# ay-lab/fithic

Measured on AMD Instinct MI355X. Metric: contact-pairs/sec through spline+p-value+BH pass (5 kb cis, whole node), higher is better.
Workload: dtype f64

## Files before the change

### fithic_amd/_capi.py

```python
import ctypes
import os
import subprocess

import numpy as np

from . import _loader

_PKG = os.path.dirname(os.path.abspath(__file__))
LIB_PATH = _loader.LIB_PATH
CSRC = os.path.join(_PKG, "csrc")

FHX_OK = 0
FHX_ERR_ARG, FHX_ERR_NO_DEVICE, FHX_ERR_HIP, FHX_ERR_UNSUPPORTED, FHX_ERR_REFERENCE_EXIT, FHX_ERR_NOMEM, FHX_ERR_INTERNAL = -1, -2, -3, -4, -5, -6, -7
MODE_INTRA_ONLY, MODE_INTER_ONLY, MODE_ALL = 0, 1, 2
TOTALS_REFERENCE, TOTALS_WIDE = 0, 1
INT64_MAX = (1 << 63) - 1

(A_HIST_SUMCC, A_HIST_NPAIRS, A_BIN_LB, A_BIN_UB, A_BIN_POSS, A_BIN_SUMCC, A_BIN_SUMDIST, A_BIN_POSS7, A_X, A_Y,
 A_KNOTS, A_COEFFS, A_TABLE_X, A_TABLE_Y0, A_TABLE_Y, A_OUTLIER_DIST_HIST, A_FDR_COUNTS, A_BIN_POSS0, A_DIST_KEYS,
 A_OUTLIER_DISTS) = range(20)
_ARRAY_DTYPE = {A_BIN_SUMDIST: np.float64, A_X: np.float64, A_Y: np.float64, A_KNOTS: np.float64,
                A_COEFFS: np.float64, A_TABLE_Y0: np.float64, A_TABLE_Y: np.float64}


# ... 71 lines not shown
    "fhx_set_skip_limit": (ctypes.c_int, [_P, ctypes.c_int64]),
    "fhx_next_pass": (ctypes.c_int, [_P, _I64P]),
    "fhx_reset_passes": (ctypes.c_int, [_P]),
    "fhx_get_stats": (ctypes.c_int, [_P, ctypes.POINTER(FhxStats)]),
    "fhx_fetch": (ctypes.c_int, [_P, _F64P, _F64P, _F64P, _F64P, _F64P]),
    "fhx_fetch_flags": (ctypes.c_int, [_P, ctypes.POINTER(ctypes.c_uint8), ctypes.POINTER(ctypes.c_uint8)]),
    "fhx_fetch_outlier_rows": (ctypes.c_int, [_P, ctypes.POINTER(ctypes.c_int64), ctypes.c_int64, ctypes.POINTER(ctypes.c_int64)]),
    "fhx_get_array": (ctypes.c_int, [_P, ctypes.c_int, _P, ctypes.c_int64, _I64P]),
    "fhx_device_ptr": (_P, [_P, ctypes.c_int]),
    "fhx_n_sorted": (ctypes.c_int64, [_P]),
    "fhx_bh_sort_stats": (ctypes.c_int, [_P, _I64P]),
    "fhx_k3_pass_info": (ctypes.c_int, [_P, _I64P]),
    "fhx_debug_k3_tiles_per_group": (ctypes.c_int, [_P, ctypes.c_int]),
    "fhx_debug_device_blocks": (ctypes.c_int, [_I64P, _I64P]),
    "fhx_debug_k1_wide": (ctypes.c_int, [_P, ctypes.c_int]),
    "fhx_k3_compact_variant": (ctypes.c_int, [_P, ctypes.POINTER(ctypes.c_int32)]),
    "fhx_kernel_seconds": (ctypes.c_int, [_P, _F64P, _F64P, _F64P]),
    "fhx_kernel_seconds_total": (ctypes.c_int, [_P, _F64P, _I64P, ctypes.c_int]),
    "fhx_kernel_events_dropped": (ctypes.c_int, [_P, _I64P]),
    "fhx_k2_heavy_launch": (ctypes.c_int, [_P, _F64P, _I64P]),
    "fhx_k2_heavy_clock": (ctypes.c_int, [_P, _F64P]),
    "fhx_k2_class_rows": (ctypes.c_int, [_P, _I64P]),
    "fhx_bdtrc_array": (ctypes.c_int, [_P, ctypes.c_double, _I32P, _F64P, ctypes.c_int64, _F64P]),
    "fhx_debug_format": (ctypes.c_int, [_P, _F64P, ctypes.c_int64, ctypes.c_int32, ctypes.c_char_p, _I32P]),
    "fhx_debug_contfrac": (ctypes.c_int, [_P, ctypes.c_int, ctypes.c_int, _F64P, _F64P, _F64P, ctypes.c_int64, _F64P]),
    "fhx_debug_lean_div": (ctypes.c_int, [_P, _F64P, _F64P, ctypes.c_int64, _F64P]),
    "fhx_debug_table_div": (ctypes.c_int, [_P, ctypes.c_int, _F64P, ctypes.c_int64, _F64P, _I32P]),
    "fhx_debug_classify": (ctypes.c_int, [_P, ctypes.c_double, _I32P, _F64P, ctypes.c_int64, _I32P, _I32P, _F64P]),
    "fhx_debug_k2_rows": (ctypes.c_int, [_P, ctypes.c_double, ctypes.c_double, _I32P, _F64P, ctypes.POINTER(ctypes.c_uint8), ctypes.c_int64,
                                         ctypes.c_int32, _F64P, _I64P, _I64P, _I64P, ctypes.c_int64]),
# ... 652 lines not shown
                        [int(v) for v in n]))

    def k3_pass_info(self):
        n = (ctypes.c_int64 * 8)()
        self._check(self._L.fhx_k3_pass_info(self._h, n))
        v = ctypes.c_int32(0)
        self._check(self._L.fhx_k3_compact_variant(self._h, ctypes.byref(v)))
        return [int(x) for x in n] + [v.value]

    def debug_k3_tiles_per_group(self, per):
        self._check(self._L.fhx_debug_k3_tiles_per_group(self._h, int(per)))

    def debug_k1_wide(self, on):
        self._check(self._L.fhx_debug_k1_wide(self._h, 1 if on else 0))

    def kernel_events_dropped(self):
        n = (ctypes.c_int64 * 4)()
        self._check(self._L.fhx_kernel_events_dropped(self._h, n))
        return list(n)

    def k2_heavy_launch(self):
        sec, rows = ctypes.c_double(0), ctypes.c_int64(0)
        self._check(self._L.fhx_k2_heavy_launch(self._h, ctypes.byref(sec), ctypes.byref(rows)))
        return sec.value, rows.value

    def k2_heavy_clock(self):
        ghz = ctypes.c_double(0)
        self._check(self._L.fhx_k2_heavy_clock(self._h, ctypes.byref(ghz)))
        return ghz.value

# ... 765 lines not shown
```

### fithic_amd/csrc/fhx_ctx.hpp

```cpp
#pragma once
#include <hip/hip_runtime.h>

#include <atomic>
#include <functional>
#include <chrono>
#include <thread>
#include <memory>
#include <sys/stat.h>
#include <unistd.h>
#include <deque>
#include <mutex>
#include <map>
#include <condition_variable>
#include <algorithm>
#include <climits>
#include <cstddef>
#include <cmath>
#include <cstdio>
#include <cstdlib>
#include <cstring>
#include <string>
#include <vector>

#include "../../include/fithic_mi355x.h"
// ... 32 lines not shown
    int32_t nslots;
    int32_t pad;
};

struct K1Sums {
    long long inter_count, inter_sum, intra_all_count, intra_all_sum, in_range_count, in_range_sum, n_skipped;
    int max_count, pad;
};

struct K2Params {
    const int32_t* loc1;
    const int32_t* loc2;
    const int32_t* count;
    const double* slot_bias;
    bool no_bias;
    const double* prior_lut;
    int lut_len;
    dev::BinomTables intra, inter;
    double inter_chr_prob;
    double outlier_thres;
    int lo_idx, hi_idx;
    int mode;
    int64_t n;
    double* p;
    unsigned long long* top_hist;
    uint8_t* outlier;
    int nonfixed;
    const int32_t* slot_mid;
    const double* table_x;
    const double* table_y;
// ... 197 lines not shown
    bool have_params = false;

    FragTable frags;
    bool have_frags = false;
    int n_chr = 0;

    std::vector<int32_t> bias_chr, bias_mid;
    std::vector<double> bias_val;
    bool have_bias = false;

    int64_t n_rows = 0;
    int32_t *d_loc1 = nullptr, *d_loc2 = nullptr, *d_count = nullptr;
    uint32_t* d_k1key = nullptr;
    bool k1key_valid = false;
    bool k1_force_wide = false;
    bool counts_integral = true;
    std::vector<ChrGrid> grid;
    ChrGrid* d_grid = nullptr;
    int16_t* d_slot_chr = nullptr;
    double* d_slot_bias = nullptr;
    int64_t n_slots = 0;
    int64_t n_dist = 0;
    bool tables_dirty = true;

    int pass_no = 0;
    uint8_t *d_skip = nullptr, *d_outlier = nullptr;
    bool skip_active = false;
    unsigned long long *d_hist_cc = nullptr, *d_hist_np = nullptr, *d_out_hist = nullptr;
    DeviceWords* d_words = nullptr;
    K1Sums* d_sums = nullptr;
// ... 140 lines not shown
    return (int)std::max<int64_t>(1, std::min<int64_t>(b, max_blocks));
}

inline int k2_classify_grid(int64_t n) {
    return grid_for(n, K2_CL_TILE, K2_MAX_SHARDS);
}
inline long long k2_shard_capacity(int64_t n) {
    const long long tiles = std::max<long long>(1, (n + K2_CL_TILE - 1) / K2_CL_TILE), grid = k2_classify_grid(n);
    return ((tiles + grid - 1) / grid) * (long long)K2_CL_TILE;
}


int build_slot_tables(fhx_ctx* ctx);
int run_ids(fhx_ctx* ctx, const unsigned long long* keys, int64_t n, unsigned int* ids, unsigned int* tile_scratch, int64_t* n_runs);
int alloc_row_arrays(fhx_ctx* ctx, int64_t n, int64_t n_dist);
int ingest_device_rows_nonfixed(fhx_ctx* ctx, const int32_t* c1, const int32_t* m1, const int32_t* c2, const int32_t* m2,
                                const int32_t* cnt, int64_t n);
int ingest_device_rows(fhx_ctx* ctx, const int32_t* c1, const int32_t* m1, const int32_t* c2, const int32_t* m2, const int32_t* cnt,
                       int64_t n);
int pass_stats_nonfixed(fhx_ctx* ctx, fhx_stats* out);
int launch_k1(fhx_ctx* ctx);
void fold_kernel_events(fhx_ctx* ctx);
void before_rerecord(fhx_ctx* ctx, int group);
K2Params make_k2_params(fhx_ctx* c);
void launch_k2_extras(fhx_ctx* ctx, const K2Params& P, int64_t n_rows, double* d_expcc, double* d_b1, double* d_b2);
int ensure_sort_scratch(fhx_ctx* ctx);
int sort_blocks_for(int64_t n_hint);
int radix_sort_pairs(fhx_ctx* ctx, unsigned long long* keys[2], unsigned int* vals[2], const unsigned long long* counter, int passes,
                     int* result_buf, int64_t n_hint = -1);
void launch_rs_scan(fhx_ctx* ctx, int nblk);
// ... 17 lines not shown
```

### fithic_amd/csrc/fhx_device.hip

```cpp
#include <thread>

#include "fhx_ctx.hpp"

extern "C" {

const char* fhx_version(void) { return "fithic-mi355x 0.2.0 (gfx950)"; }

int fhx_create(int device, fhx_ctx** out) {
    if (!out) return FHX_ERR_ARG;
    *out = nullptr;
    fhx_ctx* ctx = new (std::nothrow) fhx_ctx();
    if (!ctx) return FHX_ERR_NOMEM;
    ctx->device = device;
    if (device >= 0) {
        int count = 0;
        if (hipGetDeviceCount(&count) != hipSuccess || device >= count) {
            delete ctx;
            return FHX_ERR_NO_DEVICE;
        }
        if (hipSetDevice(device) != hipSuccess || hipStreamCreateWithFlags(&ctx->stream, hipStreamNonBlocking) != hipSuccess) {
            delete ctx;
            return FHX_ERR_HIP;
        }
        for (auto& e : ctx->ev)
// ... 25 lines not shown
void fhx_destroy(fhx_ctx* ctx) {
    if (!ctx) return;
    if (ctx->sig_sorter) fhx_destroy(ctx->sig_sorter);
    ctx->sig_sorter = nullptr;
    (void)fhx_comm_destroy(ctx);
    if (ctx->device >= 0) {
        (void)hipSetDevice(ctx->device);
        if (ctx->stream) (void)hipStreamSynchronize(ctx->stream);
        fhx_ingest_contacts_discard(ctx);
        fhx_pinned_pair_free(ctx->pinned);
        ctx->pinned = nullptr;
        dev_free(ctx->d_loc1);
        dev_free(ctx->d_loc2);
        dev_free(ctx->d_count);
        dev_free(ctx->d_k1key);
        dev_free(ctx->d_grid);
        dev_free(ctx->d_slot_chr);
        dev_free(ctx->d_slot_bias);
        dev_free(ctx->d_skip);
        dev_free(ctx->d_outlier);
        dev_free(ctx->d_grow);
        dev_free(ctx->d_hist_cc);
        dev_free(ctx->d_hist_np);
        dev_free(ctx->d_out_hist);
        dev_free(ctx->d_words);
        dev_free(ctx->d_sums);
        dev_free(ctx->d_fit_tables);
        if (ctx->h_fit_stage) (void)hipHostFree(ctx->h_fit_stage);
        if (ctx->ev_fit_copy) (void)hipEventDestroy(ctx->ev_fit_copy);
        if (ctx->ev_k3) (void)hipEventDestroy(ctx->ev_k3);
// ... 24 lines not shown
    delete ctx;
}

const char* fhx_last_error(fhx_ctx* ctx) { return ctx ? ctx->err.c_str() : "null context"; }

int fhx_set_params(fhx_ctx* ctx, const fhx_params* p) {
    if (!ctx || !p) return FHX_ERR_ARG;
    if (p->resolution < 0) return fail(ctx, FHX_ERR_ARG, "resolution must be >= 0 (0 = non-fixed-size data)");
    if (p->resolution > INT32_MAX) return fail(ctx, FHX_ERR_ARG, "resolution too large");
    if (p->n_bins <= 0 || p->mapp_thres < 0 || p->mode < 0 || p->mode > 2) return fail(ctx, FHX_ERR_ARG, "bad parameter");
    if (p->totals != FHX_TOTALS_REFERENCE && p->totals != FHX_TOTALS_WIDE) return fail(ctx, FHX_ERR_ARG, "totals must be FHX_TOTALS_REFERENCE or FHX_TOTALS_WIDE");
    if (p->bias_low > p->bias_up)
        return fail(ctx, FHX_ERR_REFERENCE_EXIT, "bias lower bound is greater than bias upper bound (fithic.py:261-263)");
    if (ctx->n_rows > 0 && ctx->have_params && p->resolution != ctx->prm.resolution)
        return fail(ctx, FHX_ERR_ARG, "the resolution cannot change after the contact rows were loaded");
    if (!ctx->have_params || p->resolution != ctx->prm.resolution || p->bias_low != ctx->prm.bias_low || p->bias_up != ctx->prm.bias_up)
        ctx->tables_dirty = true;
    ctx->prm = *p;
    ctx->nonfixed = p->resolution == 0 || ctx->offgrid;
    ctx->have_params = true;
    return FHX_OK;
}

int fhx_load_fragments(fhx_ctx* ctx, const int32_t* chr, const int32_t* mid, const int32_t* hits, int64_t n,
                       const int32_t* chr_sort_rank, int32_t n_chr) {
    if (!ctx || !chr || !mid || !hits || !chr_sort_rank || n < 0 || n_chr <= 0) return FHX_ERR_ARG;
    if (!ctx->have_params) return fail(ctx, FHX_ERR_ARG, "fhx_set_params must be called first");
    std::vector<int64_t> cnt(n_chr, 0), mx(n_chr, -1);
    std::vector<uint8_t> present(n_chr, 0);
    std::vector<std::vector<int32_t>> mids_of(ctx->nonfixed ? n_chr : 0);
    for (int64_t i = 0; i < n; ++i) {
        const int c = chr[i];
// ... 19 lines not shown
            ctx->frags.mids.push_back(std::move(mids_of[c]));
        }
    }
    ctx->n_chr = std::max(ctx->n_chr, n_chr);
    ctx->have_frags = true;
    return FHX_OK;
}

int fhx_load_bias(fhx_ctx* ctx, const int32_t* chr, const int32_t* mid, const double* bias, int64_t n) {
    if (!ctx || n < 0 || (n > 0 && (!chr || !mid || !bias))) return FHX_ERR_ARG;
    ctx->bias_chr.assign(chr, chr + n);
    ctx->bias_mid.assign(mid, mid + n);
    ctx->bias_val.assign(bias, bias + n);
    ctx->have_bias = n > 0;
    ctx->tables_dirty = true;
    return FHX_OK;
}

int fhx_load_pairs_device(fhx_ctx* ctx, const void* c1, const void* m1, const void* c2, const void* m2, const void* cnt,
                          int64_t n, void* stream) {
    if (!ctx || n < 0 || (n > 0 && (!c1 || !m1 || !c2 || !m2 || !cnt))) return FHX_ERR_ARG;
    if (ctx->device < 0) return fail(ctx, FHX_ERR_NO_DEVICE, "host-only context");
    FHX_HIP(hipSetDevice(ctx->device));
    FHX_HIP(hipStreamSynchronize((hipStream_t)stream));
    ctx->counts_integral = true;
    ctx->offgrid = false;
    ctx->nonfixed = ctx->have_params && ctx->prm.resolution == 0;
    if (ctx->have_params && ctx->nonfixed)
        return ingest_device_rows_nonfixed(ctx, (const int32_t*)c1, (const int32_t*)m1, (const int32_t*)c2, (const int32_t*)m2,
                                           (const int32_t*)cnt, n);
// ... 523 lines not shown
```

### fithic_amd/csrc/fhx_k1.hip

```cpp
#include "fhx_ctx.hpp"
#include "fhx_k1key.hpp"

namespace fhx {

__global__ void k0_extent(const int32_t* __restrict__ chr, const int32_t* __restrict__ mid, int64_t n, int res,
                          int n_chr, int32_t* __restrict__ max_idx, int32_t* __restrict__ min_off,
                          int32_t* __restrict__ max_off, int32_t* __restrict__ bad) {
    const int64_t stride = (int64_t)gridDim.x * blockDim.x;
    for (int64_t i = (int64_t)blockIdx.x * blockDim.x + threadIdx.x; i < n; i += stride) {
        const int c = chr[i];
        const int m = mid[i];
        if (c < 0 || c >= n_chr || m < 0) {
            atomicOr(bad, 1);
            continue;
        }
        const int idx = m / res, off = m - idx * res;
        const bool full = __ballot(1) == ~0ull;
        const int c0 = __shfl(c, 0, 64);
        if (full && __ballot(c != c0) == 0ull) {
            int hi = idx, lo_off = off, hi_off = off;
            for (int s = 32; s >= 1; s >>= 1) {
                hi = max(hi, __shfl_xor(hi, s, 64));
                lo_off = min(lo_off, __shfl_xor(lo_off, s, 64));
                hi_off = max(hi_off, __shfl_xor(hi_off, s, 64));
// ... 3 lines not shown
                if (lo_off < min_off[c]) atomicMin(&min_off[c], lo_off);
                if (hi_off > max_off[c]) atomicMax(&max_off[c], hi_off);
            }
        } else {
            if (idx > max_idx[c]) atomicMax(&max_idx[c], idx);
            if (off < min_off[c]) atomicMin(&min_off[c], off);
            if (off > max_off[c]) atomicMax(&max_off[c], off);
        }
    }
}

__global__ void k0_slots(const int32_t* __restrict__ chr1, const int32_t* __restrict__ mid1,
                         const int32_t* __restrict__ chr2, const int32_t* __restrict__ mid2,
                         const int32_t* __restrict__ cnt, int64_t n, int res, const ChrGrid* __restrict__ grid,
                         int32_t* __restrict__ loc1, int32_t* __restrict__ loc2, int32_t* __restrict__ count,
                         uint32_t* __restrict__ key) {
    const int64_t stride = (int64_t)gridDim.x * blockDim.x;
    for (int64_t i = (int64_t)blockIdx.x * blockDim.x + threadIdx.x; i < n; i += stride) {
        const int c1 = chr1[i], c2 = chr2[i];
        const int s1 = grid[c1].base + mid1[i] / res;
        const int s2 = grid[c2].base + mid2[i] / res;
        const int l2 = (c1 == c2) ? s2 : ~s2;
        const int c = cnt[i];
        loc1[i] = s1;
        loc2[i] = l2;
        count[i] = c;
        key[i] = k1key::pack_row(s1, l2, c);
    }
}

constexpr int K1_THREADS = 512;
constexpr int K1_LDS_BINS = 6144;

constexpr int K1_WIDE_BINS = 24576;
constexpr int K1_WIDE_THREADS = 1024;

template <int THREADS, bool WIDE, bool KEYED>
__global__ __launch_bounds__(THREADS) void k1_classify_hist(
    const int32_t* __restrict__ loc1, const int32_t* __restrict__ loc2, const int32_t* __restrict__ count,
    const uint32_t* __restrict__ key, const uint8_t* __restrict__ skip, int64_t skip_limit, const long long* __restrict__ grow, int64_t n, int lo_idx,
    int hi_idx,
    unsigned long long* __restrict__ hist_sumcc, unsigned long long* __restrict__ hist_npairs,
// ... 434 lines not shown
            const unsigned long long k = ((unsigned long long)(unsigned int)c << 32) | (unsigned int)m;
            const auto it = std::lower_bound(keys.begin(), keys.end(), k);
            if (it == keys.end() || *it != k) continue;
            const size_t s = (size_t)(it - keys.begin());
            if (seen[s]) continue;
            seen[s] = 1;
            double b = ctx->bias_val[i];
            if (b < ctx->prm.bias_low || std::isnan(b))
                b = -1;
            else if (b > ctx->prm.bias_up)
                b = -1;
            bias[s] = b;
        }
    }
    dev_free(ctx->d_slot_bias);
    FHX_HIP(dev_malloc(&ctx->d_slot_bias, bias.size() * sizeof(double)));
    FHX_HIP(hipMemcpyAsync(ctx->d_slot_bias, bias.data(), bias.size() * sizeof(double), hipMemcpyHostToDevice, ctx->stream));
    FHX_HIP(hipStreamSynchronize(ctx->stream));
    ctx->tables_dirty = false;
    return FHX_OK;
}

int build_slot_tables(fhx_ctx* ctx) {
    if (ctx->nonfixed) return build_slot_tables_nonfixed(ctx);
    const int64_t res = ctx->prm.resolution;
    std::vector<double> bias((size_t)std::max<int64_t>(ctx->n_slots, 1), ctx->have_bias ? -1.0 : 1.0);
    std::vector<int16_t> slot_chr((size_t)std::max<int64_t>(ctx->n_slots, 1), 0);
    for (size_t c = 0; c < ctx->grid.size(); ++c)
        for (int32_t s = 0; s < ctx->grid[c].nslots; ++s) slot_chr[(size_t)ctx->grid[c].base + s] = (int16_t)c;
    if (ctx->have_bias) {
// ... 6 lines not shown
            const int64_t idx = m / res;
            if (m - idx * res != g.off || idx >= g.nslots) continue;
            const size_t s = (size_t)g.base + (size_t)idx;
            if (seen[s]) continue;
            seen[s] = 1;
            double b = ctx->bias_val[i];
            if (b < ctx->prm.bias_low || std::isnan(b))
                b = -1;
            else if (b > ctx->prm.bias_up)
                b = -1;
            bias[s] = b;
        }
    }
    dev_free(ctx->d_slot_bias);
    dev_free(ctx->d_slot_chr);
    FHX_HIP(dev_malloc(&ctx->d_slot_bias, bias.size() * sizeof(double)));
    FHX_HIP(dev_malloc(&ctx->d_slot_chr, slot_chr.size() * sizeof(int16_t)));
    FHX_HIP(hipMemcpyAsync(ctx->d_slot_bias, bias.data(), bias.size() * sizeof(double), hipMemcpyHostToDevice, ctx->stream));
    FHX_HIP(hipMemcpyAsync(ctx->d_slot_chr, slot_chr.data(), slot_chr.size() * sizeof(int16_t), hipMemcpyHostToDevice,
                           ctx->stream));
    FHX_HIP(hipStreamSynchronize(ctx->stream));
    ctx->tables_dirty = false;
    return FHX_OK;
}

int run_ids(fhx_ctx* ctx, const unsigned long long* keys, int64_t n, unsigned int* ids, unsigned int* tile_scratch,
            int64_t* n_runs) {
    *n_runs = 0;
    if (n == 0) return FHX_OK;
    const int tiles = (int)((n + SEG_TILE - 1) / SEG_TILE);
    unsigned long long* total = &ctx->d_words->run_total;
    hipLaunchKernelGGL(seg_count_heads, dim3(tiles), dim3(SEG_THREADS), 0, ctx->stream, keys, n, tile_scratch);
    hipLaunchKernelGGL(seg_scan_tiles, dim3(1), dim3(1024), 0, ctx->stream, tile_scratch, (int64_t)tiles, total);
    hipLaunchKernelGGL(seg_ids, dim3(tiles), dim3(SEG_THREADS), 0, ctx->stream, keys, n, (const unsigned int*)tile_scratch, ids);
    FHX_HIP(hipGetLastError());
    unsigned long long t = 0;
    FHX_HIP(hipMemcpyAsync(&t, total, sizeof(t), hipMemcpyDeviceToHost, ctx->stream));
    FHX_HIP(hipStreamSynchronize(ctx->stream));
    *n_runs = (int64_t)t;
    return FHX_OK;
}

int alloc_row_arrays(fhx_ctx* ctx, int64_t n, int64_t n_dist);

int ingest_device_rows_nonfixed(fhx_ctx* ctx, const int32_t* c1, const int32_t* m1, const int32_t* c2, const int32_t* m2,
                                const int32_t* cnt, int64_t n) {
    if (!ctx->have_params) return fail(ctx, FHX_ERR_ARG, "fhx_set_params must be called before fhx_load_pairs");
    if (n < 0) return fail(ctx, FHX_ERR_ARG, "negative row count");
    if (2 * n >= (1ll << 32)) return fail(ctx, FHX_ERR_UNSUPPORTED, "more than 2^31 rows per GPU: shard the contacts");
    int rc = ensure_sort_scratch(ctx);
    if (rc != FHX_OK) return rc;
    const int64_t n2 = 2 * n;
    const size_t cap2 = std::max<size_t>(4, (size_t)n2);
    DeviceScratch tmp;
    unsigned long long* keys[2] = {nullptr, nullptr};
    unsigned int* vals[2] = {nullptr, nullptr};
    unsigned int *ids = nullptr, *tiles = nullptr;
    int32_t* loc = nullptr;
// ... 124 lines not shown
            n_dist = std::max<int64_t>(n_dist, (int64_t)ctx->grid[c].nslots + 1);
        }
    }
    if (base >= (1ll << 31)) return fail(ctx, FHX_ERR_UNSUPPORTED, "more than 2^31 loci");
    ctx->n_slots = base;
    ctx->n_dist = n_dist;
    dev_free(ctx->d_grid);
    FHX_HIP(dev_malloc(&ctx->d_grid, std::max<size_t>(1, ctx->grid.size()) * sizeof(ChrGrid)));
    FHX_HIP(hipMemcpyAsync(ctx->d_grid, ctx->grid.data(), ctx->grid.size() * sizeof(ChrGrid), hipMemcpyHostToDevice,
                           ctx->stream));
    {
        const int rc = alloc_row_arrays(ctx, n, n_dist);
        if (rc != FHX_OK) return rc;
    }
    mark("row arrays + workspace allocated");
    hipLaunchKernelGGL(k0_slots, dim3(blocks), dim3(256), 0, ctx->stream, c1, m1, c2, m2, cnt, n, res, ctx->d_grid,
                       ctx->d_loc1, ctx->d_loc2, ctx->d_count, ctx->d_k1key);
    FHX_HIP(hipGetLastError());
    FHX_HIP(hipStreamSynchronize(ctx->stream));
    ctx->k1key_valid = true;
    mark("locus slots");
    if (timing) std::fprintf(stderr, "fhx_load_pairs_device: %lld rows:%s\n", (long long)n, t_report.c_str());
    return FHX_OK;
}

int alloc_row_arrays(fhx_ctx* ctx, int64_t n, int64_t n_dist) {
    const size_t cap = std::max<size_t>(4, ((size_t)n + 3) / 4 * 4);
    dev_free(ctx->d_loc1);
    dev_free(ctx->d_loc2);
    dev_free(ctx->d_count);
    dev_free(ctx->d_k1key);
    ctx->k1key_valid = false;
    dev_free(ctx->d_skip);
    dev_free(ctx->d_outlier);
    dev_free(ctx->d_p);
    dev_free(ctx->d_q);
    dev_free(ctx->d_grow);
    FHX_HIP(dev_malloc(&ctx->d_loc1, cap * sizeof(int32_t)));
    FHX_HIP(dev_malloc(&ctx->d_loc2, cap * sizeof(int32_t)));
    FHX_HIP(dev_malloc(&ctx->d_count, cap * sizeof(int32_t)));
    if (!ctx->nonfixed) FHX_HIP(dev_malloc(&ctx->d_k1key, cap * sizeof(uint32_t)));
    FHX_HIP(dev_malloc(&ctx->d_skip, cap));
    FHX_HIP(dev_malloc(&ctx->d_outlier, cap));
    FHX_HIP(dev_malloc(&ctx->d_p, cap * sizeof(double)));
    FHX_HIP(dev_malloc(&ctx->d_q, cap * sizeof(double)));
    ctx->q_prefilled = false;
    FHX_HIP(hipMemsetAsync(ctx->d_skip, 0, cap, ctx->stream));
// ... 267 lines not shown
    st.in_range_sum = pk[5];
    st.max_count = pk[7];
    st.n_dist = ctx->n_dist;
    st.n_skipped = pk[6];
    ctx->have_stats = true;
    ctx->have_fit = ctx->have_bins = ctx->have_p = ctx->have_q = false;
    if (out) *out = st;
    return FHX_OK;
}

int fhx_debug_k1_wide(fhx_ctx* ctx, int on) {
    if (!ctx || on < 0 || on > 1) return FHX_ERR_ARG;
    ctx->k1_force_wide = on != 0;
    return FHX_OK;
}
```

### fithic_amd/csrc/fhx_k2.hip

```cpp
#include "fhx_ctx.hpp"

namespace fhx {

__device__ __forceinline__ double prior_by_search(const K2Params& P, long long dist) {
    double look = (double)dist;
    if (look < P.min_x) look = P.min_x;
    if (look > P.max_x) look = P.max_x;
    int lo = 0, hi = P.n_table;
    while (lo < hi) {
        const int mid = (lo + hi) >> 1;
        if (P.table_x[mid] < look)
            lo = mid + 1;
        else
            hi = mid;
    }
    return P.table_y[min(lo, P.n_table - 1)];
}

template <int NF = -1>
__device__ __forceinline__ bool row_prior(const K2Params& P, int l1, int l2, double& prior, bool& is_inter) {
    const bool inter = l2 < 0;
    const int s2 = inter ? ~l2 : l2;
    const double b1 = P.no_bias ? 1.0 : P.slot_bias[l1], b2 = P.no_bias ? 1.0 : P.slot_bias[s2];
    if ((b1 < 0 || b2 < 0) && !inter) return false;
// ... 32 lines not shown
        tab[r] = P.prior_lut[min(dist[r], P.lut_len - 1)];
    }
#pragma unroll
    for (int r = 0; r < ITEMS; ++r) {
        const bool inter = l2[r] < 0;
        const double bb = b1[r] * b2[r];
        const bool as_intra = !inter && P.mode != FHX_MODE_INTER_ONLY;
        const bool discarded = (b1[r] < 0 || b2[r] < 0) && !inter;
        const bool in_range = dist[r] >= P.lo_idx && dist[r] <= P.hi_idx;
        live[r] = !discarded && (as_intra ? in_range : P.mode != FHX_MODE_INTRA_ONLY);
        is_inter[r] = !as_intra;
        prior[r] = live[r] ? (as_intra ? tab[r] : P.inter_chr_prob) * bb : 1.0;
    }
}

constexpr int K2_HIST_BINS = 4096;
struct FusedHist {
    unsigned int* h;
    unsigned int ones;
    bool on;
    __device__ __forceinline__ void init(unsigned int* lds, const unsigned long long* global) {
        h = lds;
        ones = 0;
        on = global != nullptr;
        if (on) {
            for (int i = threadIdx.x; i < K2_HIST_BINS; i += blockDim.x) h[i] = 0;
            __syncthreads();
        }
    }
    __device__ __forceinline__ void add(double v) {
// ... 26 lines not shown
        __syncthreads();
        for (int i = threadIdx.x; i < K2_HIST_BINS; i += blockDim.x)
            if (h[i]) atomicAdd(&global[i], (unsigned long long)h[i]);
    }
};

template <bool SCATTERED>
__device__ __forceinline__ void store_p(double* dst, double v) {
    if (SCATTERED)
        __builtin_nontemporal_store(v, dst);
    else
        *dst = v;
}

constexpr int K2_TB_COUNTS = 128;
template <int NF, int WPE, int TABLE, bool HOIST = false, bool PACK = false>
__global__ __launch_bounds__(K2_THREADS) __attribute__((amdgpu_waves_per_eu(WPE, WPE))) void k2_classify(K2Params P, K2Queues Q) {
    static_assert(!HOIST || NF == 0, "the hoisted gathers are the fixed-size path's");
    static_assert(TABLE == 0 || TABLE == 3, "table variants 1 and 2 were measured and dropped");
    constexpr int ITEMS = K2_CL_ITEMS, WAVES = K2_THREADS / 64, WAVE_ROWS = 64 * ITEMS;
    __shared__ unsigned int cnt[K2_QUEUES + 1];
    __shared__ double cf_prior[WAVES][WAVE_ROWS];
    __shared__ unsigned short cf_idx[WAVES][WAVE_ROWS];
    __shared__ unsigned int hist_lds[K2_HIST_BINS];
    __shared__ unsigned int heavy_lds[K2H_BUCKETS];
    __shared__ double tb_lds[TABLE == 3 ? 2 * K2_TB_COUNTS : 1];
    if (TABLE == 3) {
        static_assert(2 * K2_TB_COUNTS <= K2_THREADS, "one thread per table entry");
        if (threadIdx.x < 2 * K2_TB_COUNTS) {
            const int c = threadIdx.x & (K2_TB_COUNTS - 1);
            const double n_total = threadIdx.x < K2_TB_COUNTS ? P.intra.n : P.inter.n;
            const double fk = (double)c - 1.0;
            const double aa = fk + 1.0, bb = n_total - fk;
// ... 7 lines not shown
    FusedHist H;
    H.init(hist_lds, P.top_hist);
    __syncthreads();
    const int lane = threadIdx.x & 63;
    const int wave = threadIdx.x >> 6;
    const unsigned long long lane_lt = (1ull << lane) - 1ull;
    const int shard = (int)blockIdx.x;
    const int64_t tiles = (P.n + K2_CL_TILE - 1) / K2_CL_TILE;
    const int4* a4 = reinterpret_cast<const int4*>(P.loc1);
    const int4* b4 = reinterpret_cast<const int4*>(P.loc2);
    const int4* c4 = reinterpret_cast<const int4*>(P.count);
    for (int64_t t = blockIdx.x; t < tiles; t += gridDim.x) {
        const int64_t wave_row0 = t * K2_CL_TILE + (int64_t)wave * WAVE_ROWS;
        const int64_t row0 = wave_row0 + lane * ITEMS;
        int l1_of[ITEMS] = {0, 0, 0, 0}, l2_of[ITEMS] = {0, 0, 0, 0}, count_of[ITEMS] = {0, 0, 0, 0};
        if (row0 < P.n) {
            const int4 a = a4[row0 >> 2], b = b4[row0 >> 2], c = c4[row0 >> 2];
            l1_of[0] = a.x; l1_of[1] = a.y; l1_of[2] = a.z; l1_of[3] = a.w;
            l2_of[0] = b.x; l2_of[1] = b.y; l2_of[2] = b.z; l2_of[3] = b.w;
            count_of[0] = c.x; count_of[1] = c.y; count_of[2] = c.z; count_of[3] = c.w;
            if (HOIST && row0 + ITEMS > P.n) {
#pragma unroll
                for (int r = 1; r < ITEMS; ++r)
                    if (row0 + r >= P.n) l1_of[r] = l2_of[r] = 0;
            }
        }
        int cls_of[ITEMS];
        double prior_of[ITEMS];
        bool inter_of[ITEMS], live_of[ITEMS];
        if (HOIST) rows_prior_fixed<ITEMS>(P, l1_of, l2_of, prior_of, inter_of, live_of);
#pragma unroll
        for (int r = 0; r < ITEMS; ++r) {
            const int64_t i = row0 + r;
            int cls = -1;
            double prior = 1.0;
            int c = count_of[r];
            if (i < P.n) {
                double pv = 1.0;
                bool is_inter = false;
                cls = 0;
                bool live;
                if (HOIST) {
                    live = live_of[r];
                    prior = prior_of[r];
                    is_inter = inter_of[r];
// ... 661 lines not shown
        const int l1 = loc1[i], l2 = loc2[i];
        const int s2 = l2 < 0 ? ~l2 : l2;
        const long long dist = llabs((long long)slot_mid[l1] - (long long)slot_mid[s2]);
        dist_list[atomicAdd(n_out, 1ull)] = (unsigned long long)dist;
    }
}


K2Params make_k2_params(fhx_ctx* c) {
    K2Params P{};
    P.loc1 = c->d_loc1;
    P.loc2 = c->d_loc2;
    P.count = c->d_count;
    P.slot_bias = c->d_slot_bias;
    P.no_bias = !c->have_bias;
    P.prior_lut = c->d_lut;
    P.lut_len = (int)std::min<size_t>(std::max<size_t>(c->fit.prior_lut.size(), 1), (size_t)INT32_MAX);
    const double n_intra = bdtrc_total(c->prm, c->stats.in_range_sum), n_inter = bdtrc_total(c->prm, c->stats.inter_sum);
    P.intra = dev::BinomTables{c->d_lbeta_intra, c->d_invb_intra, n_intra, (n_intra + 1.0) < dev::kMaxGam};
    P.inter = dev::BinomTables{c->d_lbeta_inter, c->d_invb_inter, n_inter, (n_inter + 1.0) < dev::kMaxGam};
    P.total_intra = (double)c->stats.in_range_sum;
    P.total_inter = (double)c->stats.inter_sum;
    P.inter_chr_prob = c->fit.inter_chr_prob;
    P.outlier_thres = 1.0 / c->fit.bh_total_tests;
    const int64_t res = std::max<int64_t>(c->prm.resolution, 1);
    P.lo_idx = (int)std::min<int64_t>((c->prm.dist_low + res - 1) / res, INT32_MAX);
    P.hi_idx = (int)std::min<int64_t>(c->prm.dist_up / res, INT32_MAX);
    P.mode = c->prm.mode;
    P.n = c->n_rows;
    P.p = c->d_p;
// ... 126 lines not shown
    constexpr int PIECE = (SMALL_N || CLS == dev::BC_CF_BD) ? 4 : 5;
    hipLaunchKernelGGL(HIP_KERNEL_NAME(k2_queue_by_count<CLS, SMALL_N, PIECE>), dim3(resident_grid(ctx, k2_queue_by_count<CLS, SMALL_N, PIECE>)),
                       dim3(K2_THREADS), 0, ctx->stream, P, Q.q[CLS - 1], (unsigned int*)(ctx->d_words->k2_next + CLS));
}
template <int ROWS, int WAVES, bool SMALL_N>
static void launch_k2h_heavy(fhx_ctx* ctx, const K2Params& P, QEntry* redo) {
    hipLaunchKernelGGL(HIP_KERNEL_NAME(k2h_heavy<ROWS, WAVES, SMALL_N>), dim3(256 * WAVES), dim3(K2H_THREADS), 0, ctx->stream,
                       K2HeavyParams{P.intra, P.inter, P.p, P.top_hist}, (const QEntry*)ctx->d_queue_sorted, (const unsigned int*)ctx->d_k2h_off,
                       (const unsigned int*)ctx->d_digit_total, (const dev::CfRow*)ctx->d_cf_tab, redo, &ctx->d_words->k2_redo,
                       (unsigned int*)ctx->d_words->k2_next);
}

template <bool SMALL_N>
static int launch_k2(fhx_ctx* ctx, const K2Plan& plan, const K2Params& P, const K2Queues& Q) {
    const dim3 cgrid(plan.n_shards), block(K2_THREADS);
    if (P.nonfixed)
        hipLaunchKernelGGL(HIP_KERNEL_NAME(k2_classify<1, 4, 0>), cgrid, block, 0, ctx->stream, P, Q);
    else
        hipLaunchKernelGGL(HIP_KERNEL_NAME(k2_classify<0, 4, 3, true, true>), cgrid, block, 0, ctx->stream, P, Q);
    hipLaunchKernelGGL(k2_closed, dim3(256 * 8), block, 0, ctx->stream, P, Q.q[K2_CLOSED - 1], &ctx->d_words->k2_redo, &ctx->d_words->bh_cutoff);
    if (plan.legacy_heavy) {
        FHX_HIP(hipEventRecord(ctx->ev[6], ctx->stream));
        launch_k2_queue<dev::BC_CF_SWAPPED, SMALL_N>(ctx, P, Q);
        FHX_HIP(hipEventRecord(ctx->ev[7], ctx->stream));
        ctx->ev_folded[3] = false;
        launch_k2_queue_by_count<dev::BC_CF_BD, SMALL_N>(ctx, P, Q);
        launch_k2_queue_by_count<dev::BC_CF_BCF, SMALL_N>(ctx, P, Q);
        launch_k2_queue<dev::BC_PSERIES, SMALL_N>(ctx, P, Q);
        return FHX_OK;
    }
    static_assert(K2H_BUCKETS == RADIX && K2H_BLOCKS == SORT_BLOCKS, "the radix sort's count matrix and scan are reused");
    QEntry* hq = ctx->d_queue[0];
    launch_rs_scan(ctx, (int)SORT_BLOCKS);
    hipLaunchKernelGGL(k2h_offsets_and_tables, dim3(K2H_GENERIC + 1), dim3(1024), 0, ctx->stream, (const unsigned int*)ctx->d_digit_total,
// ... 55 lines not shown
    ctx->have_q = false;
    ctx->outliers_folded = false;
    ctx->n_sorted = -1;
    return FHX_OK;
}

int fhx_pvalues(fhx_ctx* ctx) {
    if (!ctx) return FHX_ERR_ARG;
    if (ctx->device < 0) return fail(ctx, FHX_ERR_NO_DEVICE, "host-only context");
    if (!ctx->have_fit) return fail(ctx, FHX_ERR_ARG, "fhx_fit must run first");
    FHX_HIP(hipSetDevice(ctx->device));
    if (ctx->tables_dirty) {
        const int r2 = build_slot_tables(ctx);
        if (r2 != FHX_OK) return r2;
    }
    K2Params P = make_k2_params(ctx);
    before_rerecord(ctx, 1);
    FHX_HIP(hipEventRecord(ctx->ev[2], ctx->stream));
    const K2Plan plan = plan_k2(ctx, P);
    const bool prezeroed = ctx->k2_prezeroed;
    ctx->k2_prezeroed = false;
    ctx->k2_hist_valid = false;
    if (plan.memo_cap < 0) {
        const int rh = k2_fused_hist(ctx, prezeroed, &P);
        if (rh != FHX_OK) return rh;
        ctx->k2_hist_valid = true;
    }
    const K2Params P_rows = P;
    K2Memo M;
    int rc = plan.memo_cap >= 0 ? k2_table_rows(ctx, plan, &M, &P) : FHX_OK;
// ... 432 lines not shown
```

### include/fithic_mi355x.h

```cpp
#ifndef FITHIC_MI355X_H
#define FITHIC_MI355X_H

#include <stdint.h>

#ifdef __cplusplus
extern "C" {
#endif

#define FHX_OK 0
#define FHX_ERR_ARG (-1)
#define FHX_ERR_NO_DEVICE (-2)
#define FHX_ERR_HIP (-3)
#define FHX_ERR_UNSUPPORTED (-4)
#define FHX_ERR_REFERENCE_EXIT (-5)
#define FHX_ERR_NOMEM (-6)
#define FHX_ERR_INTERNAL (-7)

#define FHX_MODE_INTRA_ONLY 0
#define FHX_MODE_INTER_ONLY 1
#define FHX_MODE_ALL 2

#define FHX_TOTALS_REFERENCE 0
#define FHX_TOTALS_WIDE 1

// ... 137 lines not shown
int fhx_next_pass(fhx_ctx* ctx, int64_t* n_outliers_total);
int fhx_reset_passes(fhx_ctx* ctx);

int fhx_fetch(fhx_ctx* ctx, double* p, double* q, double* expcc, double* bias1, double* bias2);
int fhx_fetch_flags(fhx_ctx* ctx, uint8_t* outlier, uint8_t* skip);
int fhx_fetch_outlier_rows(fhx_ctx* ctx, int64_t* rows, int64_t cap, int64_t* n_out);
int fhx_get_array(fhx_ctx* ctx, int which, void* dst, int64_t capacity_elems, int64_t* n_out);
void* fhx_device_ptr(fhx_ctx* ctx, int which);
int64_t fhx_n_sorted(fhx_ctx* ctx);
int fhx_bh_sort_stats(fhx_ctx* ctx, int64_t* out8);
int fhx_k3_pass_info(fhx_ctx* ctx, int64_t* out8);
int fhx_k3_compact_variant(fhx_ctx* ctx, int32_t* out);
int fhx_debug_k3_tiles_per_group(fhx_ctx* ctx, int per);
int fhx_debug_device_blocks(int64_t* blocks, int64_t* bytes);
int fhx_debug_k1_wide(fhx_ctx* ctx, int on);
int fhx_kernel_seconds(fhx_ctx* ctx, double* k1, double* k2, double* k3);
int fhx_kernel_seconds_total(fhx_ctx* ctx, double* sums4, int64_t* counts4, int reset);
int fhx_kernel_events_dropped(fhx_ctx* ctx, int64_t* dropped4);
int fhx_k2_heavy_launch(fhx_ctx* ctx, double* seconds, int64_t* rows);
int fhx_k2_heavy_clock(fhx_ctx* ctx, double* ghz);
int fhx_k2_class_rows(fhx_ctx* ctx, int64_t* out5);

int fhx_bh_array(fhx_ctx* ctx, const double* p, int64_t n, double n_total_tests, double* q);

int fhx_bdtrc_array(fhx_ctx* ctx, double n_total, const int32_t* count, const double* prior, int64_t n, double* out);

int fhx_debug_k2_rows(fhx_ctx* ctx, double n_intra, double n_inter, const int32_t* count, const double* prior, const uint8_t* is_inter,
                      int64_t n, int32_t nonfixed, double* p_out, int64_t* class_rows5, int64_t* n_redo, int64_t* top_hist,
                      int64_t hist_cap);

// ... 270 lines not shown
```

Before: 13.91 billion.

## Stream packed row keys and precomputed bias column into K2 classify

Precomputes a per-row bias product column (built during slot ingest or lazily before K2) and has the K2 classify kernel read the packed k1 key plus this column instead of gathering loc1/loc2/count and two slot biases per row. The aim is to replace scattered slot-bias gathers and three int streams with one 32-bit key stream and one f64 stream. It costs an extra n-row f64 buffer, an extra build kernel when invalidated, and new invalidation logic tied to bias and params changes.

Measured after the change: 13.99 billion (median of 6 runs). About the same (+0.6%).

```diff
diff --git a/fithic_amd/_capi.py b/fithic_amd/_capi.py
--- a/fithic_amd/_capi.py
+++ b/fithic_amd/_capi.py
@@ -109,6 +109,8 @@
     "fhx_debug_k3_tiles_per_group": (ctypes.c_int, [_P, ctypes.c_int]),
     "fhx_debug_device_blocks": (ctypes.c_int, [_I64P, _I64P]),
     "fhx_debug_k1_wide": (ctypes.c_int, [_P, ctypes.c_int]),
+    "fhx_debug_k2_wide": (ctypes.c_int, [_P, ctypes.c_int]),
+    "fhx_debug_k2_stream_state": (ctypes.c_int, [_P, ctypes.POINTER(ctypes.c_int32), ctypes.POINTER(ctypes.c_int64)]),
     "fhx_k3_compact_variant": (ctypes.c_int, [_P, ctypes.POINTER(ctypes.c_int32)]),
     "fhx_kernel_seconds": (ctypes.c_int, [_P, _F64P, _F64P, _F64P]),
     "fhx_kernel_seconds_total": (ctypes.c_int, [_P, _F64P, _I64P, ctypes.c_int]),
@@ -791,6 +793,14 @@
     def debug_k1_wide(self, on):
         self._check(self._L.fhx_debug_k1_wide(self._h, 1 if on else 0))
 
+    def debug_k2_wide(self, on):
+        self._check(self._L.fhx_debug_k2_wide(self._h, 1 if on else 0))
+
+    def debug_k2_stream_state(self):
+        s, n = ctypes.c_int32(0), ctypes.c_int64(0)
+        self._check(self._L.fhx_debug_k2_stream_state(self._h, ctypes.byref(s), ctypes.byref(n)))
+        return bool(s.value), int(n.value)
+
     def kernel_events_dropped(self):
         n = (ctypes.c_int64 * 4)()
         self._check(self._L.fhx_kernel_events_dropped(self._h, n))
diff --git a/fithic_amd/csrc/fhx_ctx.hpp b/fithic_amd/csrc/fhx_ctx.hpp
--- a/fithic_amd/csrc/fhx_ctx.hpp
+++ b/fithic_amd/csrc/fhx_ctx.hpp
@@ -70,6 +70,8 @@
     const int32_t* count;
     const double* slot_bias;
     bool no_bias;
+    const uint32_t* row_key;
+    const double* row_bias;
     const double* prior_lut;
     int lut_len;
     dev::BinomTables intra, inter;
@@ -297,6 +299,11 @@
     uint32_t* d_k1key = nullptr;
     bool k1key_valid = false;
     bool k1_force_wide = false;
+    double* d_k2bias = nullptr;
+    bool k2bias_valid = false;
+    bool k2_force_wide = false;
+    bool k2_streamed = false;
+    int64_t k2bias_builds = 0;
     bool counts_integral = true;
     std::vector<ChrGrid> grid;
     ChrGrid* d_grid = nullptr;
@@ -467,6 +474,7 @@
 int build_slot_tables(fhx_ctx* ctx);
 int run_ids(fhx_ctx* ctx, const unsigned long long* keys, int64_t n, unsigned int* ids, unsigned int* tile_scratch, int64_t* n_runs);
 int alloc_row_arrays(fhx_ctx* ctx, int64_t n, int64_t n_dist);
+void k2bias_build(fhx_ctx* ctx);
 int ingest_device_rows_nonfixed(fhx_ctx* ctx, const int32_t* c1, const int32_t* m1, const int32_t* c2, const int32_t* m2,
                                 const int32_t* cnt, int64_t n);
 int ingest_device_rows(fhx_ctx* ctx, const int32_t* c1, const int32_t* m1, const int32_t* c2, const int32_t* m2, const int32_t* cnt,
diff --git a/fithic_amd/csrc/fhx_device.hip b/fithic_amd/csrc/fhx_device.hip
--- a/fithic_amd/csrc/fhx_device.hip
+++ b/fithic_amd/csrc/fhx_device.hip
@@ -63,6 +63,7 @@
         dev_free(ctx->d_loc2);
         dev_free(ctx->d_count);
         dev_free(ctx->d_k1key);
+        dev_free(ctx->d_k2bias);
         dev_free(ctx->d_grid);
         dev_free(ctx->d_slot_chr);
         dev_free(ctx->d_slot_bias);
@@ -117,8 +118,10 @@
         return fail(ctx, FHX_ERR_REFERENCE_EXIT, "bias lower bound is greater than bias upper bound (fithic.py:261-263)");
     if (ctx->n_rows > 0 && ctx->have_params && p->resolution != ctx->prm.resolution)
         return fail(ctx, FHX_ERR_ARG, "the resolution cannot change after the contact rows were loaded");
-    if (!ctx->have_params || p->resolution != ctx->prm.resolution || p->bias_low != ctx->prm.bias_low || p->bias_up != ctx->prm.bias_up)
+    if (!ctx->have_params || p->resolution != ctx->prm.resolution || p->bias_low != ctx->prm.bias_low || p->bias_up != ctx->prm.bias_up) {
         ctx->tables_dirty = true;
+        ctx->k2bias_valid = false;
+    }
     ctx->prm = *p;
     ctx->nonfixed = p->resolution == 0 || ctx->offgrid;
     ctx->have_params = true;
@@ -168,6 +171,7 @@
     ctx->bias_val.assign(bias, bias + n);
     ctx->have_bias = n > 0;
     ctx->tables_dirty = true;
+    ctx->k2bias_valid = false;
     return FHX_OK;
 }
 
diff --git a/fithic_amd/csrc/fhx_k1.hip b/fithic_amd/csrc/fhx_k1.hip
--- a/fithic_amd/csrc/fhx_k1.hip
+++ b/fithic_amd/csrc/fhx_k1.hip
@@ -1,5 +1,6 @@
 #include "fhx_ctx.hpp"
 #include "fhx_k1key.hpp"
+#include "fhx_k2bias.hpp"
 
 namespace fhx {
 
@@ -41,7 +42,7 @@
                          const int32_t* __restrict__ chr2, const int32_t* __restrict__ mid2,
                          const int32_t* __restrict__ cnt, int64_t n, int res, const ChrGrid* __restrict__ grid,
                          int32_t* __restrict__ loc1, int32_t* __restrict__ loc2, int32_t* __restrict__ count,
-                         uint32_t* __restrict__ key) {
+                         uint32_t* __restrict__ key, const double* __restrict__ slot_bias, double* __restrict__ bias_col) {
     const int64_t stride = (int64_t)gridDim.x * blockDim.x;
     for (int64_t i = (int64_t)blockIdx.x * blockDim.x + threadIdx.x; i < n; i += stride) {
         const int c1 = chr1[i], c2 = chr2[i];
@@ -53,6 +54,17 @@
         loc2[i] = l2;
         count[i] = c;
         key[i] = k1key::pack_row(s1, l2, c);
+        if (bias_col) bias_col[i] = k2bias::product(c1 != c2, slot_bias[s1], slot_bias[s2]);
+    }
+}
+
+__global__ void k2_bias_column(const int32_t* __restrict__ loc1, const int32_t* __restrict__ loc2, const double* __restrict__ slot_bias,
+                               int64_t n, double* __restrict__ bias_col) {
+    const int64_t stride = (int64_t)gridDim.x * blockDim.x;
+    for (int64_t i = (int64_t)blockIdx.x * blockDim.x + threadIdx.x; i < n; i += stride) {
+        const int l1 = loc1[i], l2 = loc2[i];
+        const bool inter = l2 < 0;
+        bias_col[i] = k2bias::product(inter, slot_bias[l1], slot_bias[inter ? ~l2 : l2]);
     }
 }
 
@@ -517,6 +529,7 @@
         }
     }
     dev_free(ctx->d_slot_bias);
+    ctx->k2bias_valid = false;
     FHX_HIP(dev_malloc(&ctx->d_slot_bias, bias.size() * sizeof(double)));
     FHX_HIP(hipMemcpyAsync(ctx->d_slot_bias, bias.data(), bias.size() * sizeof(double), hipMemcpyHostToDevice, ctx->stream));
     FHX_HIP(hipStreamSynchronize(ctx->stream));
@@ -553,6 +566,7 @@
     }
     dev_free(ctx->d_slot_bias);
     dev_free(ctx->d_slot_chr);
+    ctx->k2bias_valid = false;
     FHX_HIP(dev_malloc(&ctx->d_slot_bias, bias.size() * sizeof(double)));
     FHX_HIP(dev_malloc(&ctx->d_slot_chr, slot_chr.size() * sizeof(int16_t)));
     FHX_HIP(hipMemcpyAsync(ctx->d_slot_bias, bias.data(), bias.size() * sizeof(double), hipMemcpyHostToDevice, ctx->stream));
@@ -581,6 +595,7 @@
 }
 
 int alloc_row_arrays(fhx_ctx* ctx, int64_t n, int64_t n_dist);
+static bool k2bias_alloc(fhx_ctx* ctx);
 
 int ingest_device_rows_nonfixed(fhx_ctx* ctx, const int32_t* c1, const int32_t* m1, const int32_t* c2, const int32_t* m2,
                                 const int32_t* cnt, int64_t n) {
@@ -735,14 +750,46 @@
         if (rc != FHX_OK) return rc;
     }
     mark("row arrays + workspace allocated");
+    double* bias_col = nullptr;
+    if (ctx->have_bias && k2bias_alloc(ctx)) {
+        const int rc = build_slot_tables(ctx);
+        if (rc != FHX_OK) return rc;
+        bias_col = ctx->d_k2bias;
+    }
     hipLaunchKernelGGL(k0_slots, dim3(blocks), dim3(256), 0, ctx->stream, c1, m1, c2, m2, cnt, n, res, ctx->d_grid,
-                       ctx->d_loc1, ctx->d_loc2, ctx->d_count, ctx->d_k1key);
+                       ctx->d_loc1, ctx->d_loc2, ctx->d_count, ctx->d_k1key, (const double*)ctx->d_slot_bias, bias_col);
     FHX_HIP(hipGetLastError());
     FHX_HIP(hipStreamSynchronize(ctx->stream));
     ctx->k1key_valid = true;
+    if (bias_col) {
+        ctx->k2bias_valid = true;
+        ++ctx->k2bias_builds;
+    }
     mark("locus slots");
     if (timing) std::fprintf(stderr, "fhx_load_pairs_device: %lld rows:%s\n", (long long)n, t_report.c_str());
     return FHX_OK;
+}
+
+static bool k2bias_alloc(fhx_ctx* ctx) {
+    if (ctx->d_k2bias) return true;
+    if (ctx->nonfixed || !ctx->d_loc1) return false;
+    const size_t cap = std::max<size_t>(4, ((size_t)ctx->n_rows + 3) / 4 * 4);
+    if (dev_malloc(&ctx->d_k2bias, cap * sizeof(double)) != hipSuccess) {
+        (void)hipGetLastError();
+        ctx->d_k2bias = nullptr;
+        return false;
+    }
+    return true;
+}
+
+void k2bias_build(fhx_ctx* ctx) {
+    if (ctx->k2bias_valid || !ctx->have_bias || ctx->nonfixed || ctx->tables_dirty || !ctx->d_slot_bias || !ctx->k1key_valid) return;
+    if (!k2bias_alloc(ctx)) return;
+    hipLaunchKernelGGL(k2_bias_column, dim3(grid_for(ctx->n_rows, 256)), dim3(256), 0, ctx->stream, (const int32_t*)ctx->d_loc1,
+                       (const int32_t*)ctx->d_loc2, (const double*)ctx->d_slot_bias, ctx->n_rows, ctx->d_k2bias);
+    if (hipGetLastError() != hipSuccess) return;
+    ctx->k2bias_valid = true;
+    ++ctx->k2bias_builds;
 }
 
 int alloc_row_arrays(fhx_ctx* ctx, int64_t n, int64_t n_dist) {
@@ -752,6 +799,8 @@
     dev_free(ctx->d_count);
     dev_free(ctx->d_k1key);
     ctx->k1key_valid = false;
+    dev_free(ctx->d_k2bias);
+    ctx->k2bias_valid = false;
     dev_free(ctx->d_skip);
     dev_free(ctx->d_outlier);
     dev_free(ctx->d_p);
@@ -1049,3 +1098,16 @@
     ctx->k1_force_wide = on != 0;
     return FHX_OK;
 }
+
+int fhx_debug_k2_wide(fhx_ctx* ctx, int on) {
+    if (!ctx || on < 0 || on > 1) return FHX_ERR_ARG;
+    ctx->k2_force_wide = on != 0;
+    return FHX_OK;
+}
+
+int fhx_debug_k2_stream_state(fhx_ctx* ctx, int32_t* streamed, int64_t* bias_builds) {
+    if (!ctx || !streamed || !bias_builds) return FHX_ERR_ARG;
+    *streamed = ctx->k2_streamed ? 1 : 0;
+    *bias_builds = ctx->k2bias_builds;
+    return FHX_OK;
+}
diff --git a/fithic_amd/csrc/fhx_k2.hip b/fithic_amd/csrc/fhx_k2.hip
--- a/fithic_amd/csrc/fhx_k2.hip
+++ b/fithic_amd/csrc/fhx_k2.hip
@@ -1,4 +1,6 @@
 #include "fhx_ctx.hpp"
+#include "fhx_k1key.hpp"
+#include "fhx_k2bias.hpp"
 
 namespace fhx {
 
@@ -70,6 +72,40 @@
     }
 }
 
+template <int ITEMS>
+__device__ __forceinline__ void rows_prior_stream(const K2Params& P, int64_t row0, const uint32_t (&key)[ITEMS],
+                                                  const double (&bb)[ITEMS], int (&count)[ITEMS], double (&prior)[ITEMS],
+                                                  bool (&is_inter)[ITEMS], bool (&live)[ITEMS]) {
+    double tab[ITEMS];
+    int dist[ITEMS];
+    bool inter_row[ITEMS];
+#pragma unroll
+    for (int r = 0; r < ITEMS; ++r) {
+        const k1key::Row u = k1key::unpack(key[r]);
+        inter_row[r] = u.inter;
+        dist[r] = u.d;
+        count[r] = u.count;
+        if (u.escape) {
+            const int l1 = P.loc1[row0 + r], l2 = P.loc2[row0 + r];
+            const int s2 = l2 < 0 ? ~l2 : l2;
+            inter_row[r] = l2 < 0;
+            dist[r] = abs(l1 - s2);
+            count[r] = P.count[row0 + r];
+        }
+        tab[r] = P.prior_lut[min(dist[r], P.lut_len - 1)];
+    }
+#pragma unroll
+    for (int r = 0; r < ITEMS; ++r) {
+        const bool inter = inter_row[r];
+        const bool as_intra = !inter && P.mode != FHX_MODE_INTER_ONLY;
+        const bool discarded = !inter && bb[r] < 0;
+        const bool in_range = dist[r] >= P.lo_idx && dist[r] <= P.hi_idx;
+        live[r] = !discarded && (as_intra ? in_range : P.mode != FHX_MODE_INTRA_ONLY);
+        is_inter[r] = !as_intra;
+        prior[r] = live[r] ? (as_intra ? tab[r] : P.inter_chr_prob) * bb[r] : 1.0;
+    }
+}
+
 constexpr int K2_HIST_BINS = 4096;
 struct FusedHist {
     unsigned int* h;
@@ -126,9 +162,10 @@
 }
 
 constexpr int K2_TB_COUNTS = 128;
-template <int NF, int WPE, int TABLE, bool HOIST = false, bool PACK = false>
+template <int NF, int WPE, int TABLE, bool HOIST = false, bool PACK = false, bool STREAM = false>
 __global__ __launch_bounds__(K2_THREADS) __attribute__((amdgpu_waves_per_eu(WPE, WPE))) void k2_classify(K2Params P, K2Queues Q) {
     static_assert(!HOIST || NF == 0, "the hoisted gathers are the fixed-size path's");
+    static_assert(!STREAM || (HOIST && NF == 0), "the streamed rows replace the hoisted gathers");
     static_assert(TABLE == 0 || TABLE == 3, "table variants 1 and 2 were measured and dropped");
     constexpr int ITEMS = K2_CL_ITEMS, WAVES = K2_THREADS / 64, WAVE_ROWS = 64 * ITEMS;
     __shared__ unsigned int cnt[K2_QUEUES + 1];
@@ -166,7 +203,28 @@
         const int64_t wave_row0 = t * K2_CL_TILE + (int64_t)wave * WAVE_ROWS;
         const int64_t row0 = wave_row0 + lane * ITEMS;
         int l1_of[ITEMS] = {0, 0, 0, 0}, l2_of[ITEMS] = {0, 0, 0, 0}, count_of[ITEMS] = {0, 0, 0, 0};
-        if (row0 < P.n) {
+        int cls_of[ITEMS];
+        double prior_of[ITEMS];
+        bool inter_of[ITEMS], live_of[ITEMS];
+        if (STREAM) {
+            uint32_t key_of[ITEMS] = {0u, 0u, 0u, 0u};
+            double bb_of[ITEMS] = {1.0, 1.0, 1.0, 1.0};
+            if (row0 < P.n) {
+                const uint4 k = reinterpret_cast<const uint4*>(P.row_key)[row0 >> 2];
+                key_of[0] = k.x; key_of[1] = k.y; key_of[2] = k.z; key_of[3] = k.w;
+                if (!P.no_bias) {
+                    const double2 x = reinterpret_cast<const double2*>(P.row_bias)[row0 >> 1];
+                    const double2 y = reinterpret_cast<const double2*>(P.row_bias)[(row0 >> 1) + 1];
+                    bb_of[0] = x.x; bb_of[1] = x.y; bb_of[2] = y.x; bb_of[3] = y.y;
+                }
+                if (row0 + ITEMS > P.n) {
+#pragma unroll
+                    for (int r = 1; r < ITEMS; ++r)
+                        if (row0 + r >= P.n) key_of[r] = 0u;
+                }
+            }
+            rows_prior_stream<ITEMS>(P, row0, key_of, bb_of, count_of, prior_of, inter_of, live_of);
+        } else if (row0 < P.n) {
             const int4 a = a4[row0 >> 2], b = b4[row0 >> 2], c = c4[row0 >> 2];
             l1_of[0] = a.x; l1_of[1] = a.y; l1_of[2] = a.z; l1_of[3] = a.w;
             l2_of[0] = b.x; l2_of[1] = b.y; l2_of[2] = b.z; l2_of[3] = b.w;
@@ -177,10 +235,7 @@
                     if (row0 + r >= P.n) l1_of[r] = l2_of[r] = 0;
             }
         }
-        int cls_of[ITEMS];
-        double prior_of[ITEMS];
-        bool inter_of[ITEMS], live_of[ITEMS];
-        if (HOIST) rows_prior_fixed<ITEMS>(P, l1_of, l2_of, prior_of, inter_of, live_of);
+        if (HOIST && !STREAM) rows_prior_fixed<ITEMS>(P, l1_of, l2_of, prior_of, inter_of, live_of);
 #pragma unroll
         for (int r = 0; r < ITEMS; ++r) {
             const int64_t i = row0 + r;
@@ -872,6 +927,8 @@
     P.count = c->d_count;
     P.slot_bias = c->d_slot_bias;
     P.no_bias = !c->have_bias;
+    P.row_key = c->d_k1key;
+    P.row_bias = c->d_k2bias;
     P.prior_lut = c->d_lut;
     P.lut_len = (int)std::min<size_t>(std::max<size_t>(c->fit.prior_lut.size(), 1), (size_t)INT32_MAX);
     const double n_intra = bdtrc_total(c->prm, c->stats.in_range_sum), n_inter = bdtrc_total(c->prm, c->stats.inter_sum);
@@ -1028,10 +1085,17 @@
 template <bool SMALL_N>
 static int launch_k2(fhx_ctx* ctx, const K2Plan& plan, const K2Params& P, const K2Queues& Q) {
     const dim3 cgrid(plan.n_shards), block(K2_THREADS);
-    if (P.nonfixed)
+    const bool own_rows = P.loc1 == ctx->d_loc1 && P.n == ctx->n_rows && P.row_key == ctx->d_k1key && P.row_bias == ctx->d_k2bias;
+    const bool stream = !P.nonfixed && own_rows && ctx->d_k1key && ctx->k1key_valid && (P.no_bias || (ctx->d_k2bias && ctx->k2bias_valid)) &&
+                        !ctx->k2_force_wide;
+    ctx->k2_streamed = stream;
+    if (P.nonfixed) {
         hipLaunchKernelGGL(HIP_KERNEL_NAME(k2_classify<1, 4, 0>), cgrid, block, 0, ctx->stream, P, Q);
-    else
+    } else if (!stream) {
         hipLaunchKernelGGL(HIP_KERNEL_NAME(k2_classify<0, 4, 3, true, true>), cgrid, block, 0, ctx->stream, P, Q);
+    } else {
+        hipLaunchKernelGGL(HIP_KERNEL_NAME(k2_classify<0, 4, 3, true, true, true>), cgrid, block, 0, ctx->stream, P, Q);
+    }
     hipLaunchKernelGGL(k2_closed, dim3(256 * 8), block, 0, ctx->stream, P, Q.q[K2_CLOSED - 1], &ctx->d_words->k2_redo, &ctx->d_words->bh_cutoff);
     if (plan.legacy_heavy) {
         FHX_HIP(hipEventRecord(ctx->ev[6], ctx->stream));
@@ -1117,6 +1181,7 @@
         const int r2 = build_slot_tables(ctx);
         if (r2 != FHX_OK) return r2;
     }
+    k2bias_build(ctx);
     K2Params P = make_k2_params(ctx);
     before_rerecord(ctx, 1);
     FHX_HIP(hipEventRecord(ctx->ev[2], ctx->stream));
diff --git a/fithic_amd/csrc/fhx_k2bias.hpp b/fithic_amd/csrc/fhx_k2bias.hpp
--- /dev/null
+++ b/fithic_amd/csrc/fhx_k2bias.hpp
@@ -0,0 +1,23 @@
+#pragma once
+#include <cstdint>
+
+#if defined(__HIPCC__) || defined(__CUDACC__)
+#define FHX_K2BIAS_FN __host__ __device__ inline
+#else
+#define FHX_K2BIAS_FN inline
+#endif
+
+namespace fhx {
+namespace k2bias {
+
+constexpr double DISCARDED = -1.0;
+
+FHX_K2BIAS_FN double product(bool inter, double b1, double b2) {
+    if (!inter && (b1 < 0 || b2 < 0)) return DISCARDED;
+    return b1 * b2;
+}
+
+FHX_K2BIAS_FN bool discarded(bool inter, double bb) { return !inter && bb < 0; }
+
+}
+}
diff --git a/include/fithic_mi355x.h b/include/fithic_mi355x.h
--- a/include/fithic_mi355x.h
+++ b/include/fithic_mi355x.h
@@ -175,6 +175,8 @@
 int fhx_debug_k3_tiles_per_group(fhx_ctx* ctx, int per);
 int fhx_debug_device_blocks(int64_t* blocks, int64_t* bytes);
 int fhx_debug_k1_wide(fhx_ctx* ctx, int on);
+int fhx_debug_k2_wide(fhx_ctx* ctx, int on);
+int fhx_debug_k2_stream_state(fhx_ctx* ctx, int32_t* streamed, int64_t* bias_builds);
 int fhx_kernel_seconds(fhx_ctx* ctx, double* k1, double* k2, double* k3);
 int fhx_kernel_seconds_total(fhx_ctx* ctx, double* sums4, int64_t* counts4, int reset);
 int fhx_kernel_events_dropped(fhx_ctx* ctx, int64_t* dropped4);
```
